# mathisbot/homomorph-rust

Measured on AMD Instinct MI355X. Metric: homomorphic u32 ops/sec (add, mul) at d=dp=tau=128; 1/2/4/8 MI355X, higher is better.
Workload: dtype u32

## Files before the change

### homomorph-rust_amd/csrc/adder_mfma.hip

```cpp
#include <hip/hip_runtime.h>

#include "mfma_gf2.h"

namespace hm {

#ifdef HM_MFMA_PROFILE
__device__ unsigned long long *g_mfma_prof;
#define HM_PT(v) const unsigned long long v = __builtin_amdgcn_s_memtime()
#define HM_PACC(k, a, b) prof[k] += (b) - (a)
#else
#define HM_PT(v)
#define HM_PACC(k, a, b)
#endif

#ifndef HM_MFMA_PREFETCH
#define HM_MFMA_PREFETCH 3
#endif
#ifndef HM_MFMA_PREFETCH25
#define HM_MFMA_PREFETCH25 4
#endif
template <int NC> constexpr int kPrefetchOf = NC > 16 ? HM_MFMA_PREFETCH25 : NC <= 8 ? 2 : HM_MFMA_PREFETCH;
template <int NC> constexpr int kStage(int k) { return NC <= 8 ? 2 * k : 1 + 3 * k; }
template <int NC, class Side, int kPrefetch = kPrefetchOf<NC>>
__device__ __forceinline__ v16f tile_mfma(const v8i (&Af)[NC], uint32_t rb, uint32_t rbn,
                                          u32x4 (&pf)[kPrefetch], v16f acc, Side &&side) {
    static_assert(NC - kPrefetch > kStage<NC>(2), "next tile's B reads must follow its ring fill (stage 2)");
    u32x4 bq[NC];
#pragma unroll
    for (int c = 0; c < kPrefetch; ++c) bq[c] = pf[c];
#pragma unroll
    for (int c = 0; c < NC; ++c) {
        if (c + kPrefetch < NC) bq[c + kPrefetch] = lds_at<const u32x4>(rb)[2 * (c + kPrefetch)];
        else pf[c + kPrefetch - NC] = lds_at<const u32x4>(rbn)[2 * (c + kPrefetch - NC)];
        const v8i Bf = {(int)bq[c].x, (int)bq[c].y, (int)bq[c].z, (int)bq[c].w, 0, 0, 0, 0};
        acc = mfma_fp4(Af[c], Bf, acc);
        asm volatile("" : "+v"(acc)::"memory");
        if (c == kStage<NC>(0)) side(0);
        if (c == kStage<NC>(1)) side(1);
        if (c == kStage<NC>(2)) side(2);
    }
    return acc;
}

constexpr uint32_t kPhaseBytes = 16u * 32u;

#ifndef HM_REC_WAIT_YOUNG
#define HM_REC_WAIT_YOUNG 0
#endif
__device__ __forceinline__ void wait_record(int young) {
    if (!HM_REC_WAIT_YOUNG || young <= 0) asm volatile("s_waitcnt vmcnt(0)" ::: "memory");
    else if (young >= 16) asm volatile("s_waitcnt vmcnt(16)" ::: "memory");
    else if (young >= 8) asm volatile("s_waitcnt vmcnt(8)" ::: "memory");
    else if (young >= 4) asm volatile("s_waitcnt vmcnt(4)" ::: "memory");
    else if (young >= 2) asm volatile("s_waitcnt vmcnt(2)" ::: "memory");
    else asm volatile("s_waitcnt vmcnt(1)" ::: "memory");
}

__device__ __forceinline__ void sum_store(uint64_t base, uint32_t off, uint32_t v) {
    asm volatile("global_store_dword %0, %1, %2" : : "v"(off), "v"(v), "s"(base) : "memory");
}

#ifndef HM_MFMA_WPB
#define HM_MFMA_WPB kAddWavesPerBlock
#endif
constexpr int kMfmaWpb = HM_MFMA_WPB;
static_assert(kMfmaWpb <= kAddWavesPerBlock, "host LDS plan");

template <int NC>
__global__ void __launch_bounds__(64 * kMfmaWpb)
__attribute__((amdgpu_waves_per_eu(MfmaCfg<NC>::kWavesPerEU, MfmaCfg<NC>::kWavesPerEU)))
add_chain_mfma_kernel(AddArgs A) {
    kt_start(A.kt);
    using Cfg = MfmaCfg<NC>;
    constexpr int kRevWords = Cfg::kRevWords, kRsWords = Cfg::kRsWords, kRec = Cfg::kRecWords;
    extern __shared__ uint32_t lds[];
    __shared__ uint32_t stage[kMfmaWpb][2][kRec];
    uint32_t *tab = lds;
    for (uint32_t k = threadIdx.x; k < 256; k += blockDim.x) {
        uint32_t v = 0u;
#pragma unroll
        for (int t = 0; t < 8; ++t) v |= ((k >> t) & 1u) << (4 * t + 1);
        tab[k] = v;
    }
    __syncthreads();
    const int wave = (int)rfl(threadIdx.x >> 6);
    const uint64_t e = (uint64_t)blockIdx.x * (blockDim.x >> 6) + wave;
    if (e >= A.n) {
        kt_finish(A.kt);
        return;
    }
    const int lane = lane_id();
    const uint32_t L = A.nbits;
    uint32_t *Ls = lds + 256 + (size_t)wave * A.chain_lds;
    uint32_t *C = Ls + Cfg::kHalo;
    uint32_t *ring = C + A.mf_cw;
    uint32_t *RS = ring + Cfg::kRingWords;
    const uint32_t *ws = A.ws + e * A.ws_stride;
    uint64_t *po = A.out.limbs + e * A.out.stride;
    uint32_t *dout = A.out.degree + e * L;
    const uint32_t oP = A.cntX, oAB = oP + A.cntP, oD = oAB + A.cntAB;
    auto rec_word = [&](uint32_t u, uint32_t &base, uint32_t &step) {
        const uint32_t offD = L * (A.cntAB + A.cntP);
        if (u < oP) base = offD + 2 * L + u, step = A.cntX;
        else if (u < oAB) base = L * A.cntAB + (u - oP), step = A.cntP;
        else if (u < oD) base = u - oAB, step = A.cntAB;
        else if (u == oD + 1) base = offD, step = 1;
        else base = offD + L, step = 1;
    };
    uint32_t lbase, lstep, lbase2 = 0, lstep2 = 0;
    rec_word((uint32_t)lane, lbase, lstep);
    if constexpr (kRec > 64) rec_word(64u + (uint32_t)lane, lbase2, lstep2);
    const bool two = kRec > 64 && oD + 2 > 64;
    const uint64_t wsu = ((uint64_t)rfl((uint32_t)((uintptr_t)ws >> 32)) << 32) |
                         rfl((uint32_t)(uintptr_t)ws);
    auto stage_rec = [&](uint32_t i) {
        const uint32_t voff = 4u * (lbase + i * lstep);
        const uint32_t m0 = (uint32_t)(uintptr_t)&stage[wave][i & 1][0];
        asm volatile("s_mov_b32 m0, %2\n\ts_nop 0\n\tglobal_load_lds_dword %0, %1"
                     :
                     : "v"(voff), "s"(wsu), "s"(m0)
                     : "memory", "m0");
        if (two) {
            const uint32_t voff2 = 4u * (lbase2 + i * lstep2);
            asm volatile("s_mov_b32 m0, %2\n\ts_nop 0\n\tglobal_load_lds_dword %0, %1"
                         :
                         : "v"(voff2), "s"(wsu), "s"(m0 + 256u)
                         : "memory", "m0");
        }
    };
    stage_rec(0);

#ifdef HM_MFMA_PROFILE
    unsigned long long prof[4] = {0, 0, 0, 0};
#endif
    for (uint32_t k = lane; k < Cfg::kHalo + A.mf_cw; k += kWave) Ls[k] = 0u;
    for (int k = 4 * kRevWords + lane; k < kRsWords; k += kWave) RS[k] = 0u;
    wsync();
    int nc = 0;
    int degc = -1;
    int tw = -1;
    int young = 0;
    uint32_t offo = 0;
    for (uint32_t i = 0; i < L; ++i) {
        HM_PT(tw0);
        wait_record(young);
        young = 0;
        const uint32_t *rec = &stage[wave][i & 1][0];
        HM_PT(t0);
        HM_PACC(3, tw0, t0);
        if (tw < 0) {
            store_sum_x(rec, (int)A.cntX, C, nc, po + offo, A.ob.b[i], dout + i, A.status);
        } else {
            const int capw = 2 * (int)cap_of(A.ob.b[i]);
            uint32_t *so = (uint32_t *)(po + offo);
            int ldeg = -1;
            if (lane < 32) {
                const uint32_t v = (lane < (int)A.cntX ? rec[lane] : 0u) ^ C[lane];
                if (lane < capw) so[lane] = v;
                if (v) ldeg = lane * 32 + 31 - (int)__builtin_clz(v);
            }
            for (int w = tw + lane; w < capw; w += kWave) so[w] = 0u;
            int deg = wave_max_i32(ldeg);
            if (nc > 32) deg = degc;
            if (lane == 0) {
                if (deg > (int)A.ob.b[i]) flag(A.status, HM_ERR_CAPACITY);
                dout[i] = (uint32_t)max(deg, 0);
            }
        }
        offo += cap_of(A.ob.b[i]);
        HM_PT(t1);
        HM_PACC(0, t0, t1);
        if (i + 1 == L) break;
        const int np = bitwords((int)rfl(rec[oD])), nab = bitwords((int)rfl(rec[oD + 1]));
        const uint32_t *abi = rec + oAB;
        wsync();
        if (np == 0 || nc == 0) {
            const int n = max(nc, nab);
            for (int w = lane; w < n; w += kWave) C[w] = w < nab ? abi[w] : 0u;
            nc = nab;
            degc = (int)rfl(rec[oD + 1]) - 1;
            tw = -1;
            wsync();
            stage_rec(i + 1);
            continue;
        }
        const uint32_t *pi = rec + oP;
        for (int k = lane; k < 4 * kRevWords; k += kWave) {
            const int q = kRevWords - 1 - (k >> 2);
            const uint32_t rev = __builtin_bitreverse32(q < np ? pi[q] : 0u);
            RS[k] = tab[(rev >> (8 * (k & 3))) & 0xFFu];
        }
        wsync();
        stage_rec(i + 1);
        const int D = np;
        const int lane = lane_opaque(), col = lane & 31, h = lane >> 5;
        v8i Af[NC];
        const int jb = 32 * (kRevWords - D + h) - 1 - row_bit(col);
        const uint32_t rw0 = lds_opaque(lds_addr(RS) + 4u * (uint32_t)(jb >> 3));
        const uint32_t sh = 4u * (uint32_t)(jb & 7);
#pragma unroll
        for (int c = 0; c < NC; ++c) {
            const HM_LDS uint32_t *rw = lds_at<const uint32_t>(rw0) + 8 * c;
            const uint32_t w0 = rw[0], w1 = rw[1], w2 = rw[2], w3 = rw[3], w4 = rw[4];
            Af[c] = (v8i){(int)funnel(w1, w0, sh), (int)funnel(w2, w1, sh), (int)funnel(w3, w2, sh),
                          (int)funnel(w4, w3, sh), 0, 0, 0, 0};
        }
        HM_PT(t2);
        HM_PACC(1, t1, t2);
        const int nout = max(nc + np, nab);
        const int tiles = (nout + 31) >> 5;
        const uint64_t sonv = (uint64_t)(uintptr_t)(po + offo);
        const uint64_t son = ((uint64_t)rfl((uint32_t)(sonv >> 32)) << 32) | rfl((uint32_t)sonv);
        const int capn = 2 * (int)cap_of(A.ob.b[i + 1]);
        const int wlo = 32;
        int ldeg = -1;
        const int alg = (int)rfl(rec[oD]) - 1 + degc;
        const bool track = alg <= (int)rfl(rec[oD + 1]) - 1;
        v16f acc;
#pragma unroll
        for (int j = 0; j < 16; ++j) acc[j] = 8388608.0f;
        uint32_t gprev = 0u;
        const uint32_t rb0 = lds_opaque(lds_addr(ring) + 16u * (uint32_t)(col + h));
        const uint32_t put0 = lds_opaque(lds_addr(ring) + 8u * (uint32_t)lane);
        uint32_t cF = lds_opaque(lds_addr(C) + 4u * (uint32_t)(32 * (tiles - 2) - D + (lane >> 1)) +
                                 2u * (uint32_t)(lane & 1));
        uint32_t cW = lds_opaque(lds_addr(C) + 4u * (uint32_t)(32 * (tiles - 1) + col));
        const uint32_t col4 = 4u * (uint32_t)col;
        auto rbase = [&](int T) { return rb0 + kPhaseBytes * (uint32_t)(T & 3); };
        {
            constexpr int kPasses = (32 + 2 * NC + 31) / 32;
            uint32_t f0[kPasses], f1[kPasses];
#pragma unroll
            for (int p = 0; p < kPasses; ++p) {
                f0[p] = lds_at<const uint8_t>(cF)[128 * (p + 1)];
                f1[p] = lds_at<const uint8_t>(cF)[128 * (p + 1) + 1];
            }
#pragma unroll
            for (int p = 0; p < kPasses; ++p) f0[p] = tab[f0[p]], f1[p] = tab[f1[p]];
#pragma unroll
            for (int p = 0; p < kPasses; ++p) {
                const uint32_t ph = kPhaseBytes * (uint32_t)((tiles - 1 + p) & 3);
                const u32x2 fn = {f0[p], f1[p]};
                *lds_at<u32x2>(put0 + ph) = fn;
                if (ph < 16u * (uint32_t)Cfg::kMirror) *lds_at<u32x2>(put0 + ph + 16u * kMfmaRingSlots) = fn;
            }
        }
        wsync();
        constexpr int kPrefetch = kPrefetchOf<NC>;
        u32x4 pf[kPrefetch];
#pragma unroll
        for (int c = 0; c < kPrefetch; ++c) pf[c] = lds_at<const u32x4>(rbase(tiles - 1))[2 * c];
        uint32_t rb = rbase(tiles - 1);
        uint32_t abw = 0u;
        for (int T = tiles - 1; T >= 0; --T) {
            wsync();
            if constexpr (NC > 16) rb = rbase(T);
            const uint32_t ph = kPhaseBytes * (uint32_t)((T - 1) & 3);
            const uint32_t rbn = rb0 + ph;
            const uint32_t pp = put0 + ph;
            const bool mirror = ph < 16u * (uint32_t)Cfg::kMirror;
            uint32_t f0, f1;
            u32x2 fn;
            if (32 * T < nab) {
                asm volatile("" ::: "memory");
                const int W = 32 * T + (lane_opaque() & 31);
                abw = W < nab ? abi[W] : 0u;
            }
            __builtin_amdgcn_s_setprio(1);
            acc = tile_mfma<NC>(Af, rb, rbn, pf, acc, [&](int stage) {
                if (stage == 0) {
                    f0 = lds_at<const uint8_t>(cF)[0], f1 = lds_at<const uint8_t>(cF)[1];
                } else if (stage == 1) {
                    asm volatile("" : "+v"(f0), "+v"(f1));
                    fn.x = tab[f0], fn.y = tab[f1];
                } else {
                    asm volatile("" : "+v"(fn));
                    *lds_at<u32x2>(pp) = fn;
                    if (mirror) *lds_at<u32x2>(pp + 16u * kMfmaRingSlots) = fn;
                }
            });
            __builtin_amdgcn_s_setprio(0);
            const uint32_t tnow = acc_parities_hi16(acc);
            const uint32_t t = (tnow ^ gprev) >> (16 - 16 * h);
            const auto sw = __builtin_amdgcn_permlane32_swap(t, gprev, false, false);
            gprev = tnow;
            const uint32_t word = sw[0] | sw[1];
            const uint32_t v = word ^ abw;
            const bool full = T >= 1 && 32 * T + 32 <= capn;
            young += full ? 1 : 0;
            if (h == 0) {
                *lds_at<uint32_t>(cW) = v;
                const uint64_t sT = son + 128u * (uint32_t)T;
                if (full) {
                    sum_store(sT, col4, v);
                } else {
                    const int W = 32 * T + (lane_opaque() & 31);
                    if (W >= wlo && W < capn) sum_store(sT, col4, v);
                }
            }
            if (track) {
                asm volatile("" ::: "memory");
                const int Wq = 32 * T + (lane_opaque() & 31);
                if (h == 0 && v) ldeg = max(ldeg, Wq * 32 + 31 - (int)__builtin_clz(v));
            }
            rb = rbn;
            cF -= 128u;
            cW -= 128u;
        }
        const int deg = track ? wave_max_i32(ldeg) : alg;
        nc = deg >= 0 ? (deg >> 5) + 1 : 0;
        degc = deg;
        tw = 32 * tiles;
        wsync();
        HM_PT(t3);
        HM_PACC(2, t2, t3);
    }
#ifdef HM_MFMA_PROFILE
    if (lane == 0)
        for (int k = 0; k < 4; ++k) g_mfma_prof[e * 4 + k] = prof[k];
#endif
    kt_finish(A.kt);
}

int launch_add_chain_mfma(const AddArgs &a, void *stream) {
    const int wpb = kMfmaWpb;
    const uint64_t blocks = (a.n + wpb - 1) / wpb;
    const size_t lds = (256 + (size_t)a.chain_lds * wpb) * 4;
#define HM_LAUNCH_CHAIN(NCV)                                                                      \
    hipLaunchKernelGGL((add_chain_mfma_kernel<NCV>), dim3((unsigned)blocks), dim3(64 * wpb), lds,  \
                       (hipStream_t)stream, a)
    if (a.mfma == MfmaCfg<7>::kChunks) HM_LAUNCH_CHAIN(7);
    else if (a.mfma == MfmaCfg<13>::kChunks) HM_LAUNCH_CHAIN(13);
    else if (a.mfma == MfmaCfg<25>::kChunks) HM_LAUNCH_CHAIN(25);
    else return -1;
#undef HM_LAUNCH_CHAIN
    return hipGetLastError() == hipSuccess ? 0 : -1;
}

}
```

Before: 9.453 million.

## Merge P bit-reversal table build into ring prefill and batch A-fragment LDS loads

Folds the per-record RS table construction (bit-reversal of P words) into the same block as the carry ring prefill. This removes one wave barrier and lets the P-word and C-byte LDS loads be issued together before the table lookups. For small chunk counts, all A-fragment words and the B prefetch loads are issued before any funnel shifts, and the next output's bound and the record degree words are hoisted to the top of the loop. It also adds profiling timestamp hooks, which compile only under a profile flag. The aim is to cut LDS latency stalls and barrier overhead on the serial chain, at the cost of more live registers.

```diff
diff --git a/homomorph-rust_amd/csrc/adder_mfma.hip b/homomorph-rust_amd/csrc/adder_mfma.hip
--- a/homomorph-rust_amd/csrc/adder_mfma.hip
+++ b/homomorph-rust_amd/csrc/adder_mfma.hip
@@ -6,11 +6,15 @@
 
 #ifdef HM_MFMA_PROFILE
 __device__ unsigned long long *g_mfma_prof;
+__device__ unsigned long long *g_mfma_stamp;
 #define HM_PT(v) const unsigned long long v = __builtin_amdgcn_s_memtime()
 #define HM_PACC(k, a, b) prof[k] += (b) - (a)
+#define HM_STAMP(k, v)                                                                             \
+    if (stamp && lane == 0) stamp[1 + 3 * i + (k)] = (v)
 #else
 #define HM_PT(v)
 #define HM_PACC(k, a, b)
+#define HM_STAMP(k, v)
 #endif
 
 #ifndef HM_MFMA_PREFETCH
@@ -132,6 +136,10 @@
 
 #ifdef HM_MFMA_PROFILE
     unsigned long long prof[4] = {0, 0, 0, 0};
+    unsigned long long *stamp = g_mfma_stamp ? g_mfma_stamp + e * (1 + 3 * (uint64_t)L) : nullptr;
+    if (stamp && lane == 0)
+        stamp[0] = (unsigned long long)__builtin_amdgcn_s_getreg(20 | 31 << 11) << 32 |
+                   __builtin_amdgcn_s_getreg(4 | 31 << 11);
 #endif
     for (uint32_t k = lane; k < Cfg::kHalo + A.mf_cw; k += kWave) Ls[k] = 0u;
     for (int k = 4 * kRevWords + lane; k < kRsWords; k += kWave) RS[k] = 0u;
@@ -141,17 +149,24 @@
     int tw = -1;
     int young = 0;
     uint32_t offo = 0;
+    uint32_t bnext = A.ob.b[0];
     for (uint32_t i = 0; i < L; ++i) {
         HM_PT(tw0);
+        HM_STAMP(0, tw0);
         wait_record(young);
         young = 0;
         const uint32_t *rec = &stage[wave][i & 1][0];
+        const uint32_t bi = bnext;
+        const uint32_t dPv = rec[oD], dABv = rec[oD + 1];
+        bnext = A.ob.b[min(i + 1, L - 1)];
+        const int dP = (int)rfl(dPv), dAB = (int)rfl(dABv);
+        asm volatile("" : "+s"(bnext));
         HM_PT(t0);
         HM_PACC(3, tw0, t0);
         if (tw < 0) {
-            store_sum_x(rec, (int)A.cntX, C, nc, po + offo, A.ob.b[i], dout + i, A.status);
+            store_sum_x(rec, (int)A.cntX, C, nc, po + offo, bi, dout + i, A.status);
         } else {
-            const int capw = 2 * (int)cap_of(A.ob.b[i]);
+            const int capw = 2 * (int)cap_of(bi);
             uint32_t *so = (uint32_t *)(po + offo);
             int ldeg = -1;
             if (lane < 32) {
@@ -163,63 +178,35 @@
             int deg = wave_max_i32(ldeg);
             if (nc > 32) deg = degc;
             if (lane == 0) {
-                if (deg > (int)A.ob.b[i]) flag(A.status, HM_ERR_CAPACITY);
+                if (deg > (int)bi) flag(A.status, HM_ERR_CAPACITY);
                 dout[i] = (uint32_t)max(deg, 0);
             }
         }
-        offo += cap_of(A.ob.b[i]);
+        offo += cap_of(bi);
         HM_PT(t1);
         HM_PACC(0, t0, t1);
+        HM_STAMP(1, 0ull);
+        HM_STAMP(2, t1);
         if (i + 1 == L) break;
-        const int np = bitwords((int)rfl(rec[oD])), nab = bitwords((int)rfl(rec[oD + 1]));
+        const int np = bitwords(dP), nab = bitwords(dAB);
         const uint32_t *abi = rec + oAB;
         wsync();
         if (np == 0 || nc == 0) {
             const int n = max(nc, nab);
             for (int w = lane; w < n; w += kWave) C[w] = w < nab ? abi[w] : 0u;
             nc = nab;
-            degc = (int)rfl(rec[oD + 1]) - 1;
+            degc = dAB - 1;
             tw = -1;
             wsync();
             stage_rec(i + 1);
+            HM_PT(tc);
+            HM_STAMP(2, tc);
             continue;
         }
-        const uint32_t *pi = rec + oP;
-        for (int k = lane; k < 4 * kRevWords; k += kWave) {
-            const int q = kRevWords - 1 - (k >> 2);
-            const uint32_t rev = __builtin_bitreverse32(q < np ? pi[q] : 0u);
-            RS[k] = tab[(rev >> (8 * (k & 3))) & 0xFFu];
-        }
-        wsync();
-        stage_rec(i + 1);
         const int D = np;
         const int lane = lane_opaque(), col = lane & 31, h = lane >> 5;
-        v8i Af[NC];
-        const int jb = 32 * (kRevWords - D + h) - 1 - row_bit(col);
-        const uint32_t rw0 = lds_opaque(lds_addr(RS) + 4u * (uint32_t)(jb >> 3));
-        const uint32_t sh = 4u * (uint32_t)(jb & 7);
-#pragma unroll
-        for (int c = 0; c < NC; ++c) {
-            const HM_LDS uint32_t *rw = lds_at<const uint32_t>(rw0) + 8 * c;
-            const uint32_t w0 = rw[0], w1 = rw[1], w2 = rw[2], w3 = rw[3], w4 = rw[4];
-            Af[c] = (v8i){(int)funnel(w1, w0, sh), (int)funnel(w2, w1, sh), (int)funnel(w3, w2, sh),
-                          (int)funnel(w4, w3, sh), 0, 0, 0, 0};
-        }
-        HM_PT(t2);
-        HM_PACC(1, t1, t2);
         const int nout = max(nc + np, nab);
         const int tiles = (nout + 31) >> 5;
-        const uint64_t sonv = (uint64_t)(uintptr_t)(po + offo);
-        const uint64_t son = ((uint64_t)rfl((uint32_t)(sonv >> 32)) << 32) | rfl((uint32_t)sonv);
-        const int capn = 2 * (int)cap_of(A.ob.b[i + 1]);
-        const int wlo = 32;
-        int ldeg = -1;
-        const int alg = (int)rfl(rec[oD]) - 1 + degc;
-        const bool track = alg <= (int)rfl(rec[oD + 1]) - 1;
-        v16f acc;
-#pragma unroll
-        for (int j = 0; j < 16; ++j) acc[j] = 8388608.0f;
-        uint32_t gprev = 0u;
         const uint32_t rb0 = lds_opaque(lds_addr(ring) + 16u * (uint32_t)(col + h));
         const uint32_t put0 = lds_opaque(lds_addr(ring) + 8u * (uint32_t)lane);
         uint32_t cF = lds_opaque(lds_addr(C) + 4u * (uint32_t)(32 * (tiles - 2) - D + (lane >> 1)) +
@@ -228,15 +215,35 @@
         const uint32_t col4 = 4u * (uint32_t)col;
         auto rbase = [&](int T) { return rb0 + kPhaseBytes * (uint32_t)(T & 3); };
         {
+            constexpr int kTrips = (4 * kRevWords + kWave - 1) / kWave;
             constexpr int kPasses = (32 + 2 * NC + 31) / 32;
-            uint32_t f0[kPasses], f1[kPasses];
+            static_assert(kTrips * kWave <= kRsWords, "the lanes past P's image write zeros inside RS");
+            static_assert(32 + kRevWords <= kRec, "P word reads stay inside the record buffer (cntX <= 32)");
+            const uint32_t pq0 = lds_opaque(lds_addr(rec + oP));
+            const uint32_t bsh = 8u * (uint32_t)(lane & 3);
+            uint32_t pw[kTrips], f0[kPasses], f1[kPasses];
+#pragma unroll
+            for (int t = 0; t < kTrips; ++t) {
+                const int q = kRevWords - 1 - 16 * t - (lane >> 2);
+                pw[t] = lds_at<const uint32_t>(pq0)[max(q, 0)];
+            }
 #pragma unroll
             for (int p = 0; p < kPasses; ++p) {
                 f0[p] = lds_at<const uint8_t>(cF)[128 * (p + 1)];
                 f1[p] = lds_at<const uint8_t>(cF)[128 * (p + 1) + 1];
             }
 #pragma unroll
+            for (int t = 0; t < kTrips; ++t) asm volatile("" : "+v"(pw[t]));
+#pragma unroll
+            for (int t = 0; t < kTrips; ++t) {
+                const int q = kRevWords - 1 - 16 * t - (lane >> 2);
+                const uint32_t rev = __builtin_bitreverse32((uint32_t)q < (uint32_t)np ? pw[t] : 0u);
+                pw[t] = tab[(rev >> bsh) & 0xFFu];
+            }
+#pragma unroll
             for (int p = 0; p < kPasses; ++p) f0[p] = tab[f0[p]], f1[p] = tab[f1[p]];
+#pragma unroll
+            for (int t = 0; t < kTrips; ++t) RS[lane + kWave * t] = pw[t];
 #pragma unroll
             for (int p = 0; p < kPasses; ++p) {
                 const uint32_t ph = kPhaseBytes * (uint32_t)((tiles - 1 + p) & 3);
@@ -246,12 +253,57 @@
             }
         }
         wsync();
+        stage_rec(i + 1);
+        v8i Af[NC];
+        const int jb = 32 * (kRevWords - D + h) - 1 - row_bit(col);
+        const uint32_t rw0 = lds_opaque(lds_addr(RS) + 4u * (uint32_t)(jb >> 3));
+        const uint32_t sh = 4u * (uint32_t)(jb & 7);
         constexpr int kPrefetch = kPrefetchOf<NC>;
         u32x4 pf[kPrefetch];
-#pragma unroll
-        for (int c = 0; c < kPrefetch; ++c) pf[c] = lds_at<const u32x4>(rbase(tiles - 1))[2 * c];
+        if constexpr (NC <= 16) {
+            uint32_t w[NC][5];
+#pragma unroll
+            for (int c = 0; c < NC; ++c)
+#pragma unroll
+                for (int k = 0; k < 5; ++k) w[c][k] = lds_at<const uint32_t>(rw0)[8 * c + k];
+#pragma unroll
+            for (int c = 0; c < kPrefetch; ++c) pf[c] = lds_at<const u32x4>(rbase(tiles - 1))[2 * c];
+#pragma unroll
+            for (int c = 0; c < NC; ++c) {
+#pragma unroll
+                for (int k = 0; k < 5; ++k) asm volatile("" : "+v"(w[c][k]));
+            }
+#pragma unroll
+            for (int c = 0; c < NC; ++c)
+                Af[c] = (v8i){(int)funnel(w[c][1], w[c][0], sh), (int)funnel(w[c][2], w[c][1], sh),
+                              (int)funnel(w[c][3], w[c][2], sh), (int)funnel(w[c][4], w[c][3], sh), 0, 0, 0, 0};
+        } else {
+#pragma unroll
+            for (int c = 0; c < NC; ++c) {
+                const HM_LDS uint32_t *rw = lds_at<const uint32_t>(rw0) + 8 * c;
+                const uint32_t w0 = rw[0], w1 = rw[1], w2 = rw[2], w3 = rw[3], w4 = rw[4];
+                Af[c] = (v8i){(int)funnel(w1, w0, sh), (int)funnel(w2, w1, sh), (int)funnel(w3, w2, sh),
+                              (int)funnel(w4, w3, sh), 0, 0, 0, 0};
+            }
+#pragma unroll
+            for (int c = 0; c < kPrefetch; ++c) pf[c] = lds_at<const u32x4>(rbase(tiles - 1))[2 * c];
+        }
+        const uint64_t sonv = (uint64_t)(uintptr_t)(po + offo);
+        const uint64_t son = ((uint64_t)rfl((uint32_t)(sonv >> 32)) << 32) | rfl((uint32_t)sonv);
+        const int capn = 2 * (int)cap_of(bnext);
+        const int wlo = 32;
+        int ldeg = -1;
+        const int alg = dP - 1 + degc;
+        const bool track = alg <= dAB - 1;
+        v16f acc;
+#pragma unroll
+        for (int j = 0; j < 16; ++j) acc[j] = 8388608.0f;
+        uint32_t gprev = 0u;
         uint32_t rb = rbase(tiles - 1);
         uint32_t abw = 0u;
+        HM_PT(t2);
+        HM_PACC(1, t1, t2);
+        HM_STAMP(1, t2);
         for (int T = tiles - 1; T >= 0; --T) {
             wsync();
             if constexpr (NC > 16) rb = rbase(T);
@@ -314,6 +366,7 @@
         wsync();
         HM_PT(t3);
         HM_PACC(2, t2, t3);
+        HM_STAMP(2, t3);
     }
 #ifdef HM_MFMA_PROFILE
     if (lane == 0)
```

Result: no change. 9.521 million (median of 6 runs) (+0.7%).
